# aerius-labs/zksnap-circuits-halo2

Hardware: AMD Instinct MI355X
Metric: BN254 G1 MSM Mpoints/sec (higher is better)
Workload: dtype u32x9 (254-bit modular integer, radix 2^29); 1 GPU; BN254 G1 MSM, 2^20 random points/scalars per GPU (BASELINE configs[1]), point-range sharded x1, inputs resident in HBM, bases registered once (prepared fixed-base table, as under ParamsKZG::commit); points_per_gpu=1048576, parallelism=point-range shard x1 + all_gather(96 B) + fold

## Files before the change

zksnap_circuits_halo2_amd/csrc/ec.hpp:

```cpp
#pragma once
#include "fp29.hpp"

namespace zkhip {

using Fq = FqParams;

struct xyzz {
  fe X, Y, ZZ, ZZZ;
};

ZK_HD xyzz xyzz_identity() {
  xyzz r;
  r.X = fe_zero(); r.Y = fe_zero(); r.ZZ = fe_zero(); r.ZZZ = fe_zero();
  return r;
}

ZK_HD bool xyzz_is_identity(const xyzz& a) { return fe_is_zero_limbs(a.ZZ); }

ZK_HD xyzz xyzz_dbl_affine(const fe& x, const fe& y) {
  xyzz r;
  fe U = fe_dbl(y);
  fe V = fe_sqr<Fq>(U);
  fe W = fe_mul<Fq>(V, U);
  fe S = fe_mul<Fq>(x, V);
  fe XX = fe_sqr<Fq>(x);
  fe M = fe_norm(fe_add(XX, fe_dbl(XX)));
  fe MM = fe_sqr<Fq>(M);
  r.X = fe_norm(fe_sub_red(MM, fe_dbl(S), Fq::P7_S3));
  fe T = fe_sub_red(S, r.X, Fq::P10_S1);
  r.Y = fe_norm(fe_sub_red(fe_mul<Fq>(M, T), fe_mul<Fq>(W, y), Fq::P3_S1));
  r.ZZ = V;
  r.ZZZ = W;
  return r;
}

ZK_HD xyzz xyzz_dbl(const xyzz& A) {
  if (xyzz_is_identity(A)) return A;
  xyzz r;
  fe U = fe_dbl(A.Y);
  fe V = fe_sqr<Fq>(U);
  fe W = fe_mul<Fq>(V, U);
  fe S = fe_mul<Fq>(A.X, V);
  fe XX = fe_sqr<Fq>(A.X);
  fe M = fe_norm(fe_add(XX, fe_dbl(XX)));
  fe MM = fe_sqr<Fq>(M);
  r.X = fe_norm(fe_sub_red(MM, fe_dbl(S), Fq::P7_S3));
  fe T = fe_sub_red(S, r.X, Fq::P10_S1);
  r.Y = fe_norm(fe_sub_red(fe_mul<Fq>(M, T), fe_mul<Fq>(W, A.Y), Fq::P3_S1));
  r.ZZ = fe_mul<Fq>(V, A.ZZ);
  r.ZZZ = fe_mul<Fq>(W, A.ZZZ);
  return r;
}

template <bool CHAIN = false>
ZK_HD void xyzz_madd_nz(xyzz& acc, const fe& x2, const fe& y2) {
  fe U2 = fe_mul<Fq, CHAIN>(acc.ZZ, x2);
  fe S2 = fe_mul<Fq, CHAIN>(acc.ZZZ, y2);
  fe P = fe_norm(fe_sub_red(U2, acc.X, Fq::P10_S1));
  fe R = fe_norm(fe_sub_red(S2, acc.Y, Fq::P6_S1));
  fe PP = fe_sqr<Fq, CHAIN>(P);
  if (fe_mulout_is_zero<Fq>(PP)) {
    fe RR0 = fe_sqr<Fq>(R);
    if (fe_mulout_is_zero<Fq>(RR0)) {
      fe one = fe_one<Fq>();
      acc = xyzz_dbl_affine(fe_mul<Fq>(one, x2), fe_mul<Fq>(one, y2));
    } else {
      acc = xyzz_identity();
    }
    return;
  }
  fe PPP = fe_mul<Fq, CHAIN>(PP, P);
  fe Q = fe_mul<Fq, CHAIN>(PP, acc.X);
  fe RR = fe_sqr<Fq, CHAIN>(R);
  fe X3 = fe_norm(fe_sub_red(RR, fe_add(PPP, fe_dbl(Q)), Fq::P7_S3));
  fe T = fe_sub_red(Q, X3, Fq::P10_S1);
  fe Y3;
  if constexpr (CHAIN) {
    Y3 = fe_mul_add<Fq, true>(R, T, PPP, fe_neg_red(acc.Y, Fq::P6_S1));
  } else {
    Y3 = fe_norm(fe_sub_red(fe_mul<Fq>(R, T), fe_mul<Fq>(PPP, acc.Y), Fq::P3_S1));
  }
  acc.ZZ = fe_mul<Fq, CHAIN>(acc.ZZ, PP);
  acc.ZZZ = fe_mul<Fq, CHAIN>(acc.ZZZ, PPP);
  acc.X = X3;
  acc.Y = Y3;
}

template <bool CHAIN = false>
ZK_HD void xyzz_madd(xyzz& acc, const fe& x2, const fe& y2) {
  if (xyzz_is_identity(acc)) {
    fe one = fe_one<Fq>();
    acc.X = fe_mul<Fq>(one, x2);
    acc.Y = fe_mul<Fq>(one, y2);
    acc.ZZ = one;
    acc.ZZZ = one;
    return;
  }
  xyzz_madd_nz<CHAIN>(acc, x2, y2);
}

ZK_HD xyzz xyzz_add(const xyzz& A, const xyzz& B) {
  if (xyzz_is_identity(A)) return B;
  if (xyzz_is_identity(B)) return A;
  fe U1 = fe_mul<Fq>(B.ZZ, A.X);
  fe U2 = fe_mul<Fq>(A.ZZ, B.X);
  fe S1 = fe_mul<Fq>(B.ZZZ, A.Y);
  fe S2 = fe_mul<Fq>(A.ZZZ, B.Y);
  fe P = fe_norm(fe_sub_red(U2, U1, Fq::P3_S1));
  fe R = fe_norm(fe_sub_red(S2, S1, Fq::P3_S1));
  fe PP = fe_sqr<Fq>(P);
  if (fe_mulout_is_zero<Fq>(PP)) {
    fe RR0 = fe_sqr<Fq>(R);
    if (fe_mulout_is_zero<Fq>(RR0)) return xyzz_dbl(A);
    return xyzz_identity();
  }
  fe PPP = fe_mul<Fq>(PP, P);
  fe Q = fe_mul<Fq>(PP, U1);
  fe RR = fe_sqr<Fq>(R);
  xyzz r;
  r.X = fe_norm(fe_sub_red(RR, fe_add(PPP, fe_dbl(Q)), Fq::P7_S3));
  fe T = fe_sub_red(Q, r.X, Fq::P10_S1);
  r.Y = fe_norm(fe_sub_red(fe_mul<Fq>(R, T), fe_mul<Fq>(PPP, S1), Fq::P3_S1));
  r.ZZ = fe_mul<Fq>(fe_mul<Fq>(A.ZZ, B.ZZ), PP);
  r.ZZZ = fe_mul<Fq>(fe_mul<Fq>(A.ZZZ, B.ZZZ), PPP);
  return r;
}

#if defined(__HIPCC__)
struct affine_words {
  uint32_t x[8], y[8];
};

ZK_D affine_words load_affine(const uint32_t* base, size_t idx) {
  affine_words a;
  const uint4* q = reinterpret_cast<const uint4*>(base + idx * 16);
  uint4 v0 = q[0], v1 = q[1], v2 = q[2], v3 = q[3];
  a.x[0] = v0.x; a.x[1] = v0.y; a.x[2] = v0.z; a.x[3] = v0.w;
  a.x[4] = v1.x; a.x[5] = v1.y; a.x[6] = v1.z; a.x[7] = v1.w;
  a.y[0] = v2.x; a.y[1] = v2.y; a.y[2] = v2.z; a.y[3] = v2.w;
  a.y[4] = v3.x; a.y[5] = v3.y; a.y[6] = v3.z; a.y[7] = v3.w;
  return a;
}

ZK_D bool affine_is_identity(const affine_words& a) {
  uint32_t o = 0;
#pragma unroll
  for (int i = 0; i < 8; i++) o |= a.x[i] | a.y[i];
  return o == 0;
}

ZK_D bool words_zero(const uint32_t (&w)[8]) { return (w[0] | w[1] | w[2] | w[3] | w[4] | w[5] | w[6] | w[7]) == 0; }

ZK_D fe fq_plain(const fe& a) { return fe_canon_lt2p<Fq>(fe_mul<Fq>(fe_const<Fq>(Fq::RAW_ONE), a)); }

ZK_D void g1_encoding_words(const fe& x_plain, const fe& y_plain, int layout, uint32_t (&w)[8]) {
  fe_pack(x_plain, w);
  w[7] |= (y_plain.l[0] & 1u) << (layout == 0 ? 30 : 31);
}

ZK_D void store_jacobian(const xyzz& a, uint32_t* out) {
  uint32_t w[8];
  if (xyzz_is_identity(a)) {
#pragma unroll
    for (int i = 0; i < 24; i++) out[i] = 0;
    fe one = fe_one<Fq>();
    fe_to_ext<Fq>(one, w);
#pragma unroll
    for (int i = 0; i < 8; i++) out[8 + i] = w[i];
    return;
  }
  fe zz2 = fe_sqr<Fq>(a.ZZ);
  fe zzz2 = fe_sqr<Fq>(a.ZZZ);
  fe_to_ext<Fq>(fe_mul<Fq>(zz2, a.X), w);
#pragma unroll
  for (int i = 0; i < 8; i++) out[i] = w[i];
  fe_to_ext<Fq>(fe_mul<Fq>(zzz2, a.Y), w);
#pragma unroll
  for (int i = 0; i < 8; i++) out[8 + i] = w[i];
  fe_to_ext<Fq>(a.ZZZ, w);
#pragma unroll
// ... 28 lines not shown
```

zksnap_circuits_halo2_amd/csrc/fp29.hpp:

```cpp
#pragma once
#include <cstdint>
#include "bn254_constants.hpp"
#if defined(__HIPCC__)
#include <type_traits>
#include "mac_blocks.hpp"
#endif

#if defined(__HIPCC__)
#define ZK_HD __host__ __device__ __forceinline__
#define ZK_D __device__ __forceinline__
#else
#define ZK_HD inline
#define ZK_D inline
#endif

namespace zkhip {

constexpr int NL = 9;
constexpr int LB = 29;
constexpr uint32_t LMASK = (1u << LB) - 1;

struct fe {
  uint32_t l[NL];
};

ZK_HD fe fe_zero() {
  fe r;
#pragma unroll
  for (int i = 0; i < NL; i++) r.l[i] = 0;
  return r;
}

template <class P>
ZK_HD fe fe_const(const uint32_t (&c)[NL]) {
  fe r;
#pragma unroll
  for (int i = 0; i < NL; i++) r.l[i] = c[i];
  return r;
}

template <class P> ZK_HD fe fe_one() { fe r;
#pragma unroll
  for (int i = 0; i < NL; i++) r.l[i] = P::ONE[i];
  return r; }

template <bool CHAIN>
ZK_HD void fe_mac(uint64_t& acc, uint32_t x, uint32_t y) {
  acc += (uint64_t)x * y;
#if defined(__HIP_DEVICE_COMPILE__)
  if constexpr (CHAIN) asm("" : "+v"(acc));
#endif
}

#if defined(__HIPCC__)
template <int K, int END, class F>
ZK_D void static_for(F&& f) {
  if constexpr (K < END) {
    f(std::integral_constant<int, K>{});
    static_for<K + 1, END>(f);
  }
}

template <class P, bool SECOND>
ZK_D fe fe_mul_blocks(const fe& a, const fe& b, const fe& c, const fe& d) {
  uint64_t acc = 0;
  uint32_t m[NL];
  fe r;
  static_for<0, NL>([&](auto kc) {
    constexpr int k = decltype(kc)::value;
    uint32_t x[NL], y[NL];
#pragma unroll
    for (int i = 0; i <= k; i++) { x[i] = a.l[i]; y[i] = b.l[k - i]; }
    mac_vv<k + 1>(acc, x, y);
    if constexpr (SECOND) {
#pragma unroll
      for (int i = 0; i <= k; i++) { x[i] = c.l[i]; y[i] = d.l[k - i]; }
      mac_vv<k + 1>(acc, x, y);
    }
    if constexpr (k > 0) {
#pragma unroll
      for (int i = 0; i < k; i++) { x[i] = m[i]; y[i] = P::P[k - i]; }
      mac_vs<k>(acc, x, y);
    }
    m[k] = ((uint32_t)acc * P::INV) & LMASK;
    acc += (uint64_t)m[k] * P::P[0];
    acc >>= LB;
  });
  static_for<NL, 2 * NL - 1>([&](auto kc) {
    constexpr int k = decltype(kc)::value, lo = k - NL + 1, n = NL - lo;
    uint32_t x[NL], y[NL];
#pragma unroll
    for (int i = 0; i < n; i++) { x[i] = a.l[lo + i]; y[i] = b.l[k - lo - i]; }
    mac_vv<n>(acc, x, y);
    if constexpr (SECOND) {
#pragma unroll
      for (int i = 0; i < n; i++) { x[i] = c.l[lo + i]; y[i] = d.l[k - lo - i]; }
      mac_vv<n>(acc, x, y);
    }
#pragma unroll
    for (int i = 0; i < n; i++) { x[i] = m[lo + i]; y[i] = P::P[k - lo - i]; }
    mac_vs<n>(acc, x, y);
    r.l[k - NL] = (uint32_t)acc & LMASK;
    acc >>= LB;
  });
  r.l[NL - 1] = (uint32_t)acc;
  return r;
}

template <class P>
ZK_D fe fe_sqr_blocks(const fe& a) {
  uint64_t acc = 0;
  uint32_t m[NL], dbl[NL];
  fe r;
#pragma unroll
  for (int i = 0; i < NL; i++) dbl[i] = a.l[i] << 1;
  static_for<0, 2 * NL - 1>([&](auto kc) {
    constexpr int k = decltype(kc)::value, lo = k < NL ? 0 : k - NL + 1;
    constexpr int cross = (k + 1) / 2 - lo;
    uint32_t x[NL], y[NL];
    if constexpr (cross > 0) {
#pragma unroll
      for (int i = 0; i < cross; i++) { x[i] = dbl[lo + i]; y[i] = a.l[k - lo - i]; }
      mac_vv<cross>(acc, x, y);
    }
    if constexpr ((k & 1) == 0) acc += (uint64_t)a.l[k / 2] * a.l[k / 2];
    constexpr int nm = k < NL ? k : NL - lo;
// ... 151 lines not shown
ZK_HD fe fe_dbl(const fe& a) {
  fe r;
#pragma unroll
  for (int i = 0; i < NL; i++) r.l[i] = a.l[i] << 1;
  return r;
}

ZK_HD fe fe_sub_red(const fe& a, const fe& b, const uint32_t (&red)[NL]) {
  fe r;
#pragma unroll
  for (int i = 0; i < NL; i++) r.l[i] = a.l[i] + red[i] - b.l[i];
  return r;
}

ZK_HD fe fe_neg_red(const fe& b, const uint32_t (&red)[NL]) {
  fe r;
#pragma unroll
  for (int i = 0; i < NL; i++) r.l[i] = red[i] - b.l[i];
  return r;
}

ZK_HD fe fe_norm(const fe& a) {
  fe r;
  uint32_t c = 0;
#pragma unroll
  for (int i = 0; i < NL - 1; i++) {
    uint32_t t = a.l[i] + c;
    r.l[i] = t & LMASK;
    c = t >> LB;
  }
  r.l[NL - 1] = a.l[NL - 1] + c;
  return r;
}

ZK_HD bool fe_is_zero_limbs(const fe& a) {
  uint32_t o = 0;
#pragma unroll
  for (int i = 0; i < NL; i++) o |= a.l[i];
  return o == 0;
}

template <class P>
ZK_HD bool fe_mulout_is_zero(const fe& a) {
  uint32_t o = 0, e = 0;
#pragma unroll
  for (int i = 0; i < NL; i++) {
    o |= a.l[i];
    e |= a.l[i] ^ P::P[i];
  }
  return (o == 0) | (e == 0);
}

template <class P>
ZK_HD fe fe_canon_lt2p(const fe& a) {
  fe d;
  int32_t borrow = 0;
#pragma unroll
  for (int i = 0; i < NL; i++) {
    int32_t t = (int32_t)a.l[i] - (int32_t)P::P[i] + borrow;
    borrow = t >> 31;
    d.l[i] = (uint32_t)t & LMASK;
  }
  fe r;
#pragma unroll
  for (int i = 0; i < NL; i++) r.l[i] = borrow ? a.l[i] : d.l[i];
  return r;
}

template <class P>
ZK_HD fe fe_reduce_soft(const fe& x) {
  constexpr uint64_t MAGIC = (1ull << 52) / (uint64_t)(P::P[NL - 1] + 1);
  const uint32_t q = (uint32_t)(((uint64_t)x.l[NL - 1] * MAGIC) >> 52);
  fe r;
  int64_t carry = 0;
#pragma unroll
  for (int i = 0; i < NL - 1; i++) {
    int64_t v = (int64_t)x.l[i] - (int64_t)((uint64_t)q * P::P[i]) + carry;
    r.l[i] = (uint32_t)v & LMASK;
    carry = v >> LB;
  }
  r.l[NL - 1] = (uint32_t)((int64_t)x.l[NL - 1] - (int64_t)((uint64_t)q * P::P[NL - 1]) + carry);
  return r;
}

template <class P>
ZK_HD fe fe_canon_lt3p(const fe& a) { return fe_canon_lt2p<P>(fe_canon_lt2p<P>(a)); }

template <class P>
ZK_HD fe fe_canon(const fe& a) {
  fe one = fe_one<P>();
  return fe_canon_lt2p<P>(fe_mul<P>(one, a));
}

template <int SH>
ZK_HD fe fe_unpack(const uint32_t (&w)[8]) {
  fe r;
#pragma unroll
  for (int i = 0; i < NL; i++) {
    uint32_t v = 0;
#pragma unroll
    for (int j = 0; j < 8; j++) {
      const int s = 32 * j + SH - LB * i;
      if (s > -32 && s < LB) v |= (s >= 0) ? (w[j] << (s & 31)) : (w[j] >> ((-s) & 31));
    }
    r.l[i] = v & LMASK;
  }
// ... 43 lines not shown
```

zksnap_circuits_halo2_amd/csrc/mac_blocks.hpp:

```cpp
#pragma once
#include <cstdint>

namespace zkhip {

__device__ __forceinline__ void mac_vv1(uint64_t& acc, uint32_t x0, uint32_t y0) {
#if defined(__HIP_DEVICE_COMPILE__)
  asm("v_mad_u64_u32 %0, vcc, %1, %2, %0\n\t"
      : "+v"(acc) : "v"(x0), "v"(y0) : "vcc");
#else
  acc += (uint64_t)x0 * y0;
#endif
}
__device__ __forceinline__ void mac_vv2(uint64_t& acc, uint32_t x0, uint32_t y0, uint32_t x1, uint32_t y1) {
#if defined(__HIP_DEVICE_COMPILE__)
  asm("v_mad_u64_u32 %0, vcc, %1, %2, %0\n\t"
      "v_mad_u64_u32 %0, vcc, %3, %4, %0\n\t"
      : "+v"(acc) : "v"(x0), "v"(y0), "v"(x1), "v"(y1) : "vcc");
#else
  acc += (uint64_t)x0 * y0; acc += (uint64_t)x1 * y1;
#endif
}
__device__ __forceinline__ void mac_vv3(uint64_t& acc, uint32_t x0, uint32_t y0, uint32_t x1, uint32_t y1, uint32_t x2, uint32_t y2) {
#if defined(__HIP_DEVICE_COMPILE__)
  asm("v_mad_u64_u32 %0, vcc, %1, %2, %0\n\t"
      "v_mad_u64_u32 %0, vcc, %3, %4, %0\n\t"
      "v_mad_u64_u32 %0, vcc, %5, %6, %0\n\t"
      : "+v"(acc) : "v"(x0), "v"(y0), "v"(x1), "v"(y1), "v"(x2), "v"(y2) : "vcc");
#else
  acc += (uint64_t)x0 * y0; acc += (uint64_t)x1 * y1; acc += (uint64_t)x2 * y2;
#endif
}
__device__ __forceinline__ void mac_vv4(uint64_t& acc, uint32_t x0, uint32_t y0, uint32_t x1, uint32_t y1, uint32_t x2, uint32_t y2, uint32_t x3, uint32_t y3) {
#if defined(__HIP_DEVICE_COMPILE__)
  asm("v_mad_u64_u32 %0, vcc, %1, %2, %0\n\t"
      "v_mad_u64_u32 %0, vcc, %3, %4, %0\n\t"
      "v_mad_u64_u32 %0, vcc, %5, %6, %0\n\t"
      "v_mad_u64_u32 %0, vcc, %7, %8, %0\n\t"
      : "+v"(acc) : "v"(x0), "v"(y0), "v"(x1), "v"(y1), "v"(x2), "v"(y2), "v"(x3), "v"(y3) : "vcc");
#else
  acc += (uint64_t)x0 * y0; acc += (uint64_t)x1 * y1; acc += (uint64_t)x2 * y2; acc += (uint64_t)x3 * y3;
#endif
}
__device__ __forceinline__ void mac_vv5(uint64_t& acc, uint32_t x0, uint32_t y0, uint32_t x1, uint32_t y1, uint32_t x2, uint32_t y2, uint32_t x3, uint32_t y3, uint32_t x4, uint32_t y4) {
#if defined(__HIP_DEVICE_COMPILE__)
  asm("v_mad_u64_u32 %0, vcc, %1, %2, %0\n\t"
      "v_mad_u64_u32 %0, vcc, %3, %4, %0\n\t"
      "v_mad_u64_u32 %0, vcc, %5, %6, %0\n\t"
      "v_mad_u64_u32 %0, vcc, %7, %8, %0\n\t"
      "v_mad_u64_u32 %0, vcc, %9, %10, %0\n\t"
      : "+v"(acc) : "v"(x0), "v"(y0), "v"(x1), "v"(y1), "v"(x2), "v"(y2), "v"(x3), "v"(y3), "v"(x4), "v"(y4) : "vcc");
#else
  acc += (uint64_t)x0 * y0; acc += (uint64_t)x1 * y1; acc += (uint64_t)x2 * y2; acc += (uint64_t)x3 * y3; acc += (uint64_t)x4 * y4;
#endif
}
__device__ __forceinline__ void mac_vv6(uint64_t& acc, uint32_t x0, uint32_t y0, uint32_t x1, uint32_t y1, uint32_t x2, uint32_t y2, uint32_t x3, uint32_t y3, uint32_t x4, uint32_t y4, uint32_t x5, uint32_t y5) {
#if defined(__HIP_DEVICE_COMPILE__)
  asm("v_mad_u64_u32 %0, vcc, %1, %2, %0\n\t"
// ... 195 lines not shown
```

zksnap_circuits_halo2_amd/csrc/msm.hip:

```cpp
#include <hip/hip_runtime.h>
#include <atomic>
#include <cstdint>
#include <cstdio>
#include <cstring>
#include <cstdlib>
#include <mutex>
#include "ec_quad.hpp"
#include "fe_inverse.hpp"
#include "msm_digits.hpp"
#include "reduce_plan.hpp"
#include "zkhip_internal.hpp"

namespace zkhip {

static inline size_t align_up(size_t v, size_t a) { return (v + a - 1) / a * a; }

constexpr int FINE_BITS = 12;
constexpr int MAX_GROUPS = 128;
constexpr int MAX_WIDE_W = 16;
static int msm_narrow_windows(int c, int W) {
  if (c <= 16) return 0;
  const int narrow = W * c - 256;
  return narrow > 0 && narrow <= W ? narrow : 0;
}
// ... 837 lines not shown
      if (nfull > head) pos = atomicAdd(&joff[ORDER_JMAX], nfull - head);
      const uint32_t st = s0 + ((nt - 1) << task_shift);
      order[atomicAdd(&lh[rem], 1u)] = make_uint4(nt == 1 ? (0x80000000u | k) : t + nt - 1, st, rem, sorted[st]);
      if (tasks) tasks[t + nt - 1] = task_t{k, st, rem};
      if (tasks && nt > seq_parts) {
        const uint32_t P = (nt + HEAVY_SLICE - 1) / HEAVY_SLICE;
        const uint32_t idx = atomicAdd(heavy_count, P);
        for (uint32_t i = 0; i < P; i++)
          if (idx + i < heavy_cap) heavy[idx + i] = make_uint2(k, i);
      }
      mx = max(mx, nt);
    }
    const bool coop = nfull - head > COOP_TASKS;
    if (!coop) {
      for (uint32_t j = head; j < nfull; j++) {
        const uint32_t st = s0 + (j << task_shift);
        order[pos + j - head] = make_uint4(t + j, st, full, sorted[st]);
        if (tasks) tasks[t + j] = task_t{k, st, full};
      }
    }
    unsigned long long big = __ballot(coop);
    while (big) {
      const int src = __ffsll((long long)big) - 1;
      big &= big - 1;
      const uint32_t bt = (uint32_t)__shfl((int)t, src, 64), bs0 = (uint32_t)__shfl((int)s0, src, 64), bpos = (uint32_t)__shfl((int)pos, src, 64),
                     bnfull = (uint32_t)__shfl((int)nfull, src, 64), bhead = (uint32_t)__shfl((int)head, src, 64);
      for (uint32_t j = bhead + lane; j < bnfull; j += 64) {
        const uint32_t st = bs0 + (j << task_shift);
        order[bpos + j - bhead] = make_uint4(bt + j, st, full, sorted[st]);
        if (tasks) tasks[bt + j] = task_t{base + (uint32_t)src, st, full};
      }
    }
  }
  if (tasks) {
#pragma unroll
    for (int off = 32; off >= 1; off >>= 1) mx = max(mx, (uint32_t)__shfl_xor((int)mx, off, 64));
    if (lane == 0 && mx > 1) atomicMax(max_parts, mx);
  }
}

template <bool TABLE>
__global__ void __launch_bounds__(128) __attribute__((amdgpu_waves_per_eu(4, 4))) k_accumulate(const task_t* __restrict__ tasks, const uint32_t* __restrict__ ntasks_p,
                                                    const uint4* __restrict__ order, const uint32_t* __restrict__ sorted,
                                                    const uint32_t* __restrict__ bases, uint32_t* __restrict__ partials,
                                                    uint32_t* __restrict__ buckets, const uint32_t* __restrict__ bases2, uint32_t split) {
  auto point = [&](uint32_t idx) -> affine_words {
    if constexpr (!TABLE) { if (idx >= split) return load_affine(bases2, idx - split); }
    return load_affine(bases, idx);
  };
  const uint32_t ntasks = *ntasks_p;
  for (uint32_t i = blockIdx.x * blockDim.x + threadIdx.x; i < ntasks; i += gridDim.x * blockDim.x) {
    const uint4 rec = order[i];
    const uint32_t t = rec.x;
    struct { uint32_t start, len; } tk = {rec.y, rec.z};
    xyzz acc = xyzz_identity();
    const uint32_t* refs = sorted + tk.start;
    uint32_t ref = rec.w;
    affine_words pt = point(ref & 0x7fffffffu);
    uint32_t j = 0;
    if constexpr (TABLE) {
      if (!affine_is_identity(pt)) {
        acc.X = fe_unpack<0>(pt.x);
        acc.Y = fe_unpack<0>(pt.y);
        if (ref >> 31) acc.Y = fe_norm(fe_neg_red(acc.Y, Fq::P2_S1));
        acc.ZZ = acc.ZZZ = fe_one<Fq>();
      }
      if (tk.len > 1) {
        ref = refs[1];
        pt = point(ref & 0x7fffffffu);
      }
      j = 1;
    }
    uint32_t nref = j + 1 < tk.len ? refs[j + 1] : 0u;
    for (; j < tk.len; j++) {
      affine_words cur = pt;
      uint32_t cref = ref;
      if (j + 1 < tk.len) {
        ref = nref;
        pt = point(ref & 0x7fffffffu);
      }
      if (j + 2 < tk.len) nref = refs[j + 2];
      if (affine_is_identity(cur)) continue;
      fe x2, y2;
      if constexpr (TABLE) {
        x2 = fe_unpack<0>(cur.x);
        y2 = fe_unpack<0>(cur.y);
        if (cref >> 31) y2 = fe_neg_red(y2, Fq::P2_S1);
      } else {
        x2 = fe_from_ext_lazy(cur.x);
        y2 = fe_from_ext_lazy(cur.y);
        if (cref >> 31) y2 = fe_neg_red(y2, Fq::P64_S1);
      }
      xyzz_madd<true>(acc, x2, y2);
    }
    if (t >> 31) store_xyzz(buckets, t & 0x7fffffffu, acc);
    else store_xyzz(partials, t, acc);
  }
}

constexpr uint32_t HEAVY_WGS = 256;
constexpr uint32_t HEAVY_QUAD_MAX = 256;

__device__ __forceinline__ xyzz workgroup_sum_128(xyzz acc, uint32_t* __restrict__ xch) {
#pragma unroll 1
  for (uint32_t half = 64; half >= 1; half >>= 1) {
    __syncthreads();
    if (threadIdx.x >= half && threadIdx.x < 2 * half) store_xyzz(xch, threadIdx.x - half, acc);
    __syncthreads();
    if (threadIdx.x < half) acc = xyzz_add(acc, load_xyzz(xch, threadIdx.x));
  }
  return acc;
}

__device__ __forceinline__ void combine_heavy_buckets(uint32_t wg, const uint32_t* __restrict__ task_off, uint32_t* __restrict__ partials,
                                                      uint32_t* __restrict__ buckets, const uint32_t* __restrict__ heavy_count,
                                                      const uint2* __restrict__ heavy, uint32_t heavy_cap, uint32_t* __restrict__ heavy_done,
                                                      uint32_t* __restrict__ xch , uint32_t quad_max) {
  __shared__ uint32_t is_last;
  const uint32_t nh = min(*heavy_count, heavy_cap);
  for (uint32_t i = wg; i < nh; i += HEAVY_WGS) {
    const uint2 e = heavy[i];
    const uint32_t k = e.x, sl = e.y, t = task_off[k], m = task_off[k + 1] - t;
    const uint32_t P = (m + HEAVY_SLICE - 1) / HEAVY_SLICE, lo = sl * HEAVY_SLICE, hi = min(m, lo + HEAVY_SLICE);
    if (m <= quad_max) {
      const uint32_t q = threadIdx.x & 3, quad = threadIdx.x >> 2;
      xyzz acc = xyzz_identity();
#pragma unroll 1
      for (uint32_t j = quad; j < m; j += 32) acc = xyzz_add_quad(acc, load_xyzz(partials, t + j), q);
#pragma unroll 1
      for (int mask = 4; mask < 64; mask <<= 1) acc = xyzz_add_quad(acc, xyzz_shfl_xor(acc, mask), q);
      __syncthreads();
      if (threadIdx.x == 64) store_xyzz(xch, 0, acc);
      __syncthreads();
      if (threadIdx.x < 4) {
        acc = xyzz_add_quad(acc, load_xyzz(xch, 0), q);
        if (q == 0) store_xyzz(buckets, k, acc);
      }
      continue;
    }
    xyzz acc = xyzz_identity();
#pragma unroll 1
    for (uint32_t j = lo + threadIdx.x; j < hi; j += 128) acc = xyzz_add(acc, load_xyzz(partials, t + j));
    acc = workgroup_sum_128(acc, xch);
    if (P == 1) {
      if (threadIdx.x == 0) store_xyzz(buckets, k, acc);
      continue;
    }
// ... 821 lines not shown
  fe inv = fq_inverse(pref);
  for (uint32_t ii = cnt; ii-- > 0;) {
    const xyzz Q = load_xyzz(tmp_pts, lo + ii);
    uint32_t* o = out + (size_t)(lo + ii) * 16;
    if (xyzz_is_identity(Q)) {
#pragma unroll
      for (int t = 0; t < 16; t++) o[t] = 0;
      continue;
    }
    const fe pre = load_fe9_generic(tmp_pref, lo + ii);
    const fe winv = fe_mul<Fq>(inv, pre);
    inv = fe_mul<Fq>(inv, fe_mul<Fq>(Q.ZZ, Q.ZZZ));
    const fe x = fe_mul<Fq>(fe_mul<Fq>(winv, Q.ZZZ), Q.X);
    const fe y = fe_mul<Fq>(fe_mul<Fq>(winv, Q.ZZ), Q.Y);
    uint32_t wx[8], wy[8];
    fe_to_ext<Fq>(x, wx);
    fe_to_ext<Fq>(y, wy);
#pragma unroll
    for (int t = 0; t < 8; t++) { o[t] = wx[t]; o[8 + t] = wy[t]; }
  }
}

size_t g1_fixed_base_table_bytes() { return (size_t)FIXED_W * FIXED_B * 64; }
size_t g1_fixed_base_workspace(size_t n) {
  const size_t a = g1_gen_walk_workspace(FIXED_B), b = align_up(n * 144, 256) + align_up(n * 36, 256);
  return (a > b ? a : b) + 256;
}

int g1_fixed_base_table_build(uint32_t* d_table, void* ws, size_t ws_bytes, hipStream_t stream) {
  for (int w = 0; w < FIXED_W; w++) {
    uint32_t step[8];
    fr_pow2_montgomery(16 * w, step);
    int rc = g1_gen_walk_device(step, step, FIXED_B, d_table + (size_t)w * FIXED_B * 16, ws, ws_bytes, stream);
    if (rc != ZKHIP_OK) return rc;
  }
  return ZKHIP_OK;
}

int g1_fixed_base_mul_device(const uint32_t* d_scalars, size_t n, const uint32_t* d_table, uint32_t* d_out, void* ws, size_t ws_bytes, hipStream_t stream) {
  if (n == 0) return ZKHIP_OK;
  if (n >= (1ull << 31)) { set_error("fixed_base_mul: n too large"); return ZKHIP_EINVAL; }
  if (ws_bytes < g1_fixed_base_workspace(n)) { set_error("fixed_base_mul: workspace too small"); return ZKHIP_EINVAL; }
  char* p = (char*)ws;
  uint32_t* tmp_pts = (uint32_t*)p; p += align_up(n * 144, 256);
  uint32_t* tmp_pref = (uint32_t*)p;
  const uint32_t threads = (uint32_t)((n + FIXED_CHUNK - 1) / FIXED_CHUNK);
  hipLaunchKernelGGL(k_fixed_base_mul, dim3((threads + 63) / 64), dim3(64), 0, stream, d_scalars, (uint32_t)n, d_table, d_out, tmp_pts, tmp_pref);
  HIPCHK(hipGetLastError());
  return ZKHIP_OK;
}

__device__ __forceinline__ void store_table_point(uint32_t* table, size_t idx, const fe& x, const fe& y) {
  uint32_t wx[8], wy[8];
  fe_pack(fe_canon_lt2p<Fq>(x), wx);
  fe_pack(fe_canon_lt2p<Fq>(y), wy);
  uint4* q = reinterpret_cast<uint4*>(table + idx * 16);
  q[0] = make_uint4(wx[0], wx[1], wx[2], wx[3]); q[1] = make_uint4(wx[4], wx[5], wx[6], wx[7]);
  q[2] = make_uint4(wy[0], wy[1], wy[2], wy[3]); q[3] = make_uint4(wy[4], wy[5], wy[6], wy[7]);
}

__global__ void __launch_bounds__(64) k_build_table(const uint32_t* __restrict__ bases, uint32_t n, int c, int W,
                                                    uint32_t* __restrict__ table, uint32_t* __restrict__ tmp_pts,
                                                    uint32_t* __restrict__ tmp_pref, int narrow) {
  const win_layout lay{c, W, narrow};
  const uint32_t i = blockIdx.x * blockDim.x + threadIdx.x;
  if (i >= n) return;
  affine_words pt = load_affine(bases, i);
  if (affine_is_identity(pt)) {
    for (int w = 0; w < W; w++) {
      uint4* q = reinterpret_cast<uint4*>(table + ((size_t)w * n + i) * 16);
      q[0] = q[1] = q[2] = q[3] = make_uint4(0, 0, 0, 0);
    }
    return;
  }
  xyzz P = xyzz_identity();
  xyzz_madd(P, fe_from_ext_lazy(pt.x), fe_from_ext_lazy(pt.y));
  store_table_point(table, i, P.X, P.Y);
  fe pref = fe_one<Fq>();
  for (int w = 1; w < W; w++) {
    for (int k = 0, nd = win_bits(lay, w - 1); k < nd; k++) P = xyzz_dbl(P);
    store_xyzz(tmp_pts, (size_t)(w - 1) * n + i, P);
    store_fe9_generic(tmp_pref, (size_t)(w - 1) * n + i, pref);
    pref = fe_mul<Fq>(pref, fe_mul<Fq>(P.ZZ, P.ZZZ));
  }
  fe inv = fq_inverse(pref);
  for (int w = W - 1; w >= 1; w--) {
    xyzz Q = load_xyzz(tmp_pts, (size_t)(w - 1) * n + i);
    fe pre = load_fe9_generic(tmp_pref, (size_t)(w - 1) * n + i);
    fe winv = fe_mul<Fq>(inv, pre);
    inv = fe_mul<Fq>(inv, fe_mul<Fq>(Q.ZZ, Q.ZZZ));
    fe x = fe_mul<Fq>(fe_mul<Fq>(winv, Q.ZZZ), Q.X);
    fe y = fe_mul<Fq>(fe_mul<Fq>(winv, Q.ZZ), Q.Y);
    store_table_point(table, (size_t)w * n + i, x, y);
  }
}

int prepare_bases_device(const uint32_t* d_bases, size_t n, hipStream_t stream, prepared_bases** out, int c_override, size_t n_whole) {
  if (n == 0 || n >= (1ull << 27)) { set_error("prepare_bases: n = %zu out of range", n); return ZKHIP_EINVAL; }
  const int c = c_override > 0 ? c_override : msm_pick_window_prepared(n);
  if (c < 2 || c > MAX_WINDOW_PREPARED) { set_error("prepare_bases: window bits %d out of range [2,%d]", c, MAX_WINDOW_PREPARED); return ZKHIP_EINVAL; }
  const int W = (256 + c - 1) / c;
  prepared_bases* pb = new prepared_bases();
  pb->n = n; pb->c = c; pb->W = W; pb->table = nullptr; pb->direct = nullptr;
  void *table = nullptr, *tmp = nullptr;
  const size_t tbytes = (size_t)W * n * 64, tmp_pts = align_up((size_t)(W - 1) * n * 144, 256), tmp_pref = align_up((size_t)(W - 1) * n * 36, 256);
  if (hipMalloc(&table, tbytes) != hipSuccess) { delete pb; set_error("prepare_bases: hipMalloc(%zu) failed", tbytes); return ZKHIP_ENOMEM; }
  if (hipMalloc(&tmp, tmp_pts + tmp_pref) != hipSuccess) { (void)hipFree(table); delete pb; set_error("prepare_bases: hipMalloc(%zu) failed", tmp_pts + tmp_pref); return ZKHIP_ENOMEM; }
  hipLaunchKernelGGL(k_build_table, dim3((unsigned)((n + 63) / 64)), dim3(64), 0, stream, d_bases, (uint32_t)n, c, W, (uint32_t*)table,
                     (uint32_t*)tmp, (uint32_t*)((char*)tmp + tmp_pts), msm_narrow_windows(c, W));
  hipError_t e = hipGetLastError();
  if (e == hipSuccess) e = hipStreamSynchronize(stream);
  (void)hipFree(tmp);
  if (e != hipSuccess) { (void)hipFree(table); delete pb; set_error("prepare_bases: %s", hipGetErrorString(e)); return ZKHIP_EHIP; }
  pb->table = (uint32_t*)table;
  if (c_override <= 0 && msm_direct_wanted(std::max(n, n_whole)) && prepare_direct_table(pb, d_bases, stream) != ZKHIP_OK) pb->direct = nullptr;
  *out = pb;
  return ZKHIP_OK;
}

size_t direct_table_bytes(size_t n);
static std::atomic<size_t> g_direct_bytes{0};

void release_prepared(prepared_bases* pb) {
  if (!pb) return;
  if (pb->table) (void)hipFree(pb->table);
  if (pb->direct) { (void)hipFree(pb->direct); g_direct_bytes -= direct_table_bytes(pb->n); }
  delete pb;
}

constexpr int DIRECT_W = 32, DIRECT_M = 128;

__global__ void __launch_bounds__(64) k_direct_build(const uint32_t* __restrict__ wtable , uint32_t n_all,
                                                     uint32_t i0, uint32_t cnt, uint32_t* __restrict__ direct, uint32_t* __restrict__ tmp_pts,
                                                     uint32_t* __restrict__ tmp_pref) {
  const uint32_t tid = blockIdx.x * blockDim.x + threadIdx.x, T = cnt * DIRECT_W;
  if (tid >= T) return;
  const uint32_t i = i0 + tid / DIRECT_W, w = tid % DIRECT_W;
  const affine_words pt = load_affine(wtable, (size_t)w * n_all + i);
  uint4* const slot = reinterpret_cast<uint4*>(direct + ((size_t)i * DIRECT_W + w) * DIRECT_M * 16);
  if (affine_is_identity(pt)) {
    for (int k = 0; k < DIRECT_M * 4; k++) slot[k] = make_uint4(0, 0, 0, 0);
    return;
  }
  slot[0] = make_uint4(pt.x[0], pt.x[1], pt.x[2], pt.x[3]); slot[1] = make_uint4(pt.x[4], pt.x[5], pt.x[6], pt.x[7]);
  slot[2] = make_uint4(pt.y[0], pt.y[1], pt.y[2], pt.y[3]); slot[3] = make_uint4(pt.y[4], pt.y[5], pt.y[6], pt.y[7]);
  const fe x = fe_unpack<0>(pt.x), y = fe_unpack<0>(pt.y);
  xyzz acc = xyzz_identity();
  xyzz_madd(acc, x, y);
  fe pref = fe_one<Fq>();
  for (int k = 2; k <= DIRECT_M; k++) {
    xyzz_madd(acc, x, y);
    store_xyzz(tmp_pts, (size_t)(k - 2) * T + tid, acc);
    store_fe9_generic(tmp_pref, (size_t)(k - 2) * T + tid, pref);
    pref = fe_mul<Fq>(pref, fe_mul<Fq>(acc.ZZ, acc.ZZZ));
  }
  fe inv = fq_inverse(pref);
  for (int k = DIRECT_M; k >= 2; k--) {
    const xyzz Q = load_xyzz(tmp_pts, (size_t)(k - 2) * T + tid);
    const fe pre = load_fe9_generic(tmp_pref, (size_t)(k - 2) * T + tid);
    const fe winv = fe_mul<Fq>(inv, pre);
    inv = fe_mul<Fq>(inv, fe_mul<Fq>(Q.ZZ, Q.ZZZ));
    store_table_point(direct, ((size_t)i * DIRECT_W + w) * DIRECT_M + (k - 1), fe_mul<Fq>(fe_mul<Fq>(winv, Q.ZZZ), Q.X), fe_mul<Fq>(fe_mul<Fq>(winv, Q.ZZ), Q.Y));
  }
}

template <int WPT>
__device__ __forceinline__ void direct_accumulate_body(const uint32_t* __restrict__ scalars, uint32_t n, uint32_t off,
                                                       const uint32_t* __restrict__ direct, uint32_t* __restrict__ partials) {
  constexpr uint32_t GROUPS = DIRECT_W / WPT;
  constexpr int WORDS = WPT >= 4 ? WPT / 4 : 1;
  constexpr int PER = WPT >= 4 ? 4 : WPT;
  const uint32_t tid = blockIdx.x * blockDim.x + threadIdx.x;
  if (tid >= n * GROUPS) return;
  const uint32_t i = tid / GROUPS, g = tid % GROUPS;
  uint32_t w[8];
  load_words(scalars + (size_t)i * 8, w);
  fe c32;
#pragma unroll
  for (int k = 0; k < NL; k++) c32.l[k] = FrParams::FROM_EXT_CANON[k];
  fe sv = fe_canon_lt2p<FrParams>(fe_mul<FrParams>(c32, fe_unpack<0>(w)));
  fe_pack(sv, w);
  uint32_t carry = 0;
  const uint32_t first = g * WPT;
#pragma unroll
  for (int wi = 0; wi < 8; wi++) {
#pragma unroll
    for (int b = 0; b < 4; b++) {
      const uint32_t win = (uint32_t)(wi * 4 + b);
      const uint32_t v = ((w[wi] >> (8 * b)) & 255u) + carry;
      if (win < first) carry = v >= 128u ? 1u : 0u;
    }
  }
  xyzz acc = xyzz_identity();
  static_for<0, WORDS>([&](auto hc) {
    constexpr int h = decltype(hc)::value;
    const uint32_t word = first / 4 + h, byte0 = WPT >= 4 ? 0u : first % 4;
    uint32_t own = 0;
#pragma unroll
    for (int wi = 0; wi < 8; wi++) own = ((uint32_t)wi == word) ? w[wi] : own;
    int32_t dg[PER];
#pragma unroll
    for (int b = 0; b < PER; b++) {
      const uint32_t v = ((own >> (8 * (byte0 + b))) & 255u) + carry;
      if (v >= 128u) { dg[b] = (int32_t)v - 256; carry = 1; } else { dg[b] = (int32_t)v; carry = 0; }
    }
    affine_words pts[PER];
    static_for<0, PER>([&](auto bc) {
      constexpr int b = decltype(bc)::value;
      const uint32_t mag = (uint32_t)(dg[b] < 0 ? -dg[b] : dg[b]);
      const size_t idx = (((size_t)(off + i) * DIRECT_W + first + PER * h + b) * DIRECT_M) + (mag ? mag - 1 : 0);
      pts[b] = load_affine(direct, idx);
    });
    static_for<0, PER>([&](auto bc) {
      constexpr int b = decltype(bc)::value;
      if (dg[b] != 0 && !affine_is_identity(pts[b])) {
        fe x2 = fe_unpack<0>(pts[b].x), y2 = fe_unpack<0>(pts[b].y);
        if (dg[b] < 0) y2 = fe_neg_red(y2, Fq::P2_S1);
        if (xyzz_is_identity(acc)) { acc.X = x2; acc.Y = dg[b] < 0 ? fe_norm(y2) : y2; acc.ZZ = acc.ZZZ = fe_one<Fq>(); }
        else xyzz_madd_nz<true>(acc, x2, y2);
      }
    });
  });
  store_xyzz(partials, tid, acc);
}
static inline int direct_wpt(size_t n) {
  if (n <= 1024) return 1;
  if (n <= 2048) return 2;
  if (n <= 4096) return 4;
  if (n <= 8192) return 2;
  if (n <= 16384) return 4;
  return 8;
}
#define ZK_DIRECT_KERNEL(W, OCC_LO, OCC_HI)                                                                                                          \
  __global__ void __launch_bounds__(128) __attribute__((amdgpu_waves_per_eu(OCC_LO, OCC_HI))) k_direct_accumulate##W(                                 \
      const uint32_t* __restrict__ scalars, uint32_t n, uint32_t off, const uint32_t* __restrict__ direct, uint32_t* __restrict__ partials) {         \
    direct_accumulate_body<W>(scalars, n, off, direct, partials);                                                                                     \
  }
ZK_DIRECT_KERNEL(1, 4, 4)
ZK_DIRECT_KERNEL(2, 4, 4)
ZK_DIRECT_KERNEL(4, 4, 4)
ZK_DIRECT_KERNEL(8, 2, 3)
#undef ZK_DIRECT_KERNEL

__global__ void __launch_bounds__(512) k_points_sum_quad(const uint32_t* __restrict__ in, uint32_t m, uint32_t S, uint32_t* __restrict__ out,
                                                         uint32_t* __restrict__ jac_out) {
  __shared__ __attribute__((aligned(16))) uint32_t xch[8 * 36];
  const uint32_t q = threadIdx.x & 3, quad = threadIdx.x >> 2, wave = threadIdx.x >> 6;
  const uint32_t base = blockIdx.x * 128u * S;
  xyzz acc = xyzz_identity();
#pragma unroll 1
  for (uint32_t s_ = 0; s_ < S; s_++) {
    const uint32_t idx = base + s_ * 128u + quad;
    if (idx < m) acc = xyzz_add_quad(acc, load_xyzz(in, idx), q);
  }
#pragma unroll 1
  for (int mask = 4; mask < 64; mask <<= 1) acc = xyzz_add_quad(acc, xyzz_shfl_xor(acc, mask), q);
  if ((threadIdx.x & 63) == 0) store_xyzz(xch, wave, acc);
  __syncthreads();
  if (wave == 0) {
    acc = (quad < 8) ? load_xyzz(xch, quad) : xyzz_identity();
#pragma unroll 1
    for (int mask = 4; mask < 32; mask <<= 1) acc = xyzz_add_quad(acc, xyzz_shfl_xor(acc, mask), q);
    if (threadIdx.x == 0) {
      if (jac_out) store_jacobian(acc, jac_out);
      else store_xyzz(out, blockIdx.x, acc);
    }
  }
}
// ... 252 lines not shown
```

Measured before the change: 778.6 Mpoints/s.

## Use sign-flipping mixed addition and an identity-flag bit in bucket accumulation

Bucket accumulation now uses a sign-flip formulation. The accumulator's Y is kept negated on alternate steps, so R becomes an addition and Y3 folds into a single fused mul_add without a negation. The sign is fixed once at the end. Table points now mark identity with a flag bit in the top word, replacing a 16-word OR test, and the degenerate-case zero check does a cheap one-limb early exit. The first MAC in the product uses a no-accumulator variant, and constant one is materialised with inline moves. The loop is split into a fast path and a general fallback, which adds code size and register-pressure risk.

```diff
diff --git a/zksnap_circuits_halo2_amd/csrc/ec.hpp b/zksnap_circuits_halo2_amd/csrc/ec.hpp
--- a/zksnap_circuits_halo2_amd/csrc/ec.hpp
+++ b/zksnap_circuits_halo2_amd/csrc/ec.hpp
@@ -17,18 +17,19 @@
 
 ZK_HD bool xyzz_is_identity(const xyzz& a) { return fe_is_zero_limbs(a.ZZ); }
 
+template <bool CHAIN = false>
 ZK_HD xyzz xyzz_dbl_affine(const fe& x, const fe& y) {
   xyzz r;
   fe U = fe_dbl(y);
-  fe V = fe_sqr<Fq>(U);
-  fe W = fe_mul<Fq>(V, U);
-  fe S = fe_mul<Fq>(x, V);
-  fe XX = fe_sqr<Fq>(x);
+  fe V = fe_sqr<Fq, CHAIN>(U);
+  fe W = fe_mul<Fq, CHAIN>(V, U);
+  fe S = fe_mul<Fq, CHAIN>(x, V);
+  fe XX = fe_sqr<Fq, CHAIN>(x);
   fe M = fe_norm(fe_add(XX, fe_dbl(XX)));
-  fe MM = fe_sqr<Fq>(M);
+  fe MM = fe_sqr<Fq, CHAIN>(M);
   r.X = fe_norm(fe_sub_red(MM, fe_dbl(S), Fq::P7_S3));
   fe T = fe_sub_red(S, r.X, Fq::P10_S1);
-  r.Y = fe_norm(fe_sub_red(fe_mul<Fq>(M, T), fe_mul<Fq>(W, y), Fq::P3_S1));
+  r.Y = fe_norm(fe_sub_red(fe_mul<Fq, CHAIN>(M, T), fe_mul<Fq, CHAIN>(W, y), Fq::P3_S1));
   r.ZZ = V;
   r.ZZZ = W;
   return r;
@@ -86,6 +87,38 @@
   acc.Y = Y3;
 }
 
+ZK_HD bool xyzz_madd_flip_fast(xyzz& acc, const fe& x2, const fe& y2) {
+  fe U2 = fe_mul<Fq, true>(acc.ZZ, x2);
+  fe S2 = fe_mul<Fq, true>(acc.ZZZ, y2);
+  fe P = fe_norm(fe_sub_red(U2, acc.X, Fq::P10_S1));
+  fe R = fe_norm(fe_add(S2, acc.Y));
+  fe PP = fe_sqr<Fq, true>(P);
+  if (fe_mulout_is_zero_rare<Fq>(PP)) return false;
+  fe PPP = fe_mul<Fq, true>(PP, P);
+  fe ZZ3 = fe_mul<Fq, true>(acc.ZZ, PP);
+  fe Q = fe_mul<Fq, true>(PP, acc.X);
+  fe ZZZ3 = fe_mul<Fq, true>(acc.ZZZ, PPP);
+  fe RR = fe_sqr<Fq, true>(R);
+  fe X3 = fe_norm(fe_sub_red(RR, fe_add(PPP, fe_dbl(Q)), Fq::P7_S3));
+  fe T = fe_sub_red(Q, X3, Fq::P10_S1);
+  fe Y3 = fe_mul_add<Fq, true>(R, T, PPP, acc.Y);
+  acc.ZZ = ZZ3;
+  acc.ZZZ = ZZZ3;
+  acc.X = X3;
+  acc.Y = Y3;
+  return true;
+}
+
+ZK_HD void xyzz_madd_flip_nz(xyzz& acc, const fe& x2, const fe& y2) {
+  if (xyzz_madd_flip_fast(acc, x2, y2)) return;
+  fe R = fe_norm(fe_add(fe_mul<Fq, true>(acc.ZZZ, y2), acc.Y));
+  if (fe_mulout_is_zero<Fq>(fe_sqr<Fq, true>(R))) {
+    acc = xyzz_dbl_affine<true>(x2, fe_norm(y2));
+  } else {
+    acc = xyzz_identity();
+  }
+}
+
 template <bool CHAIN = false>
 ZK_HD void xyzz_madd(xyzz& acc, const fe& x2, const fe& y2) {
   if (xyzz_is_identity(acc)) {
@@ -126,6 +159,48 @@
   return r;
 }
 
+constexpr uint32_t TABLE_POINT_IDENTITY = 1u << 31;
+
+ZK_HD void table_point_pack(const fe& x, const fe& y, uint32_t (&wx)[8], uint32_t (&wy)[8]) {
+  fe_pack(fe_canon_lt2p<Fq>(x), wx);
+  fe_pack(fe_canon_lt2p<Fq>(y), wy);
+}
+
+ZK_HD void table_point_pack_identity(uint32_t (&wx)[8], uint32_t (&wy)[8]) {
+#pragma unroll
+  for (int i = 0; i < 8; i++) wx[i] = wy[i] = 0;
+  wx[7] = TABLE_POINT_IDENTITY;
+}
+
+ZK_HD bool table_point_is_identity(const uint32_t (&wx)[8]) { return (wx[7] & TABLE_POINT_IDENTITY) != 0; }
+
+ZK_HD void xyzz_flip_copy(xyzz& acc, uint32_t sgn, const fe& x, const fe& y, uint32_t neg) {
+  acc.X = x;
+  acc.Y = (neg ^ sgn) ? fe_norm(fe_neg_red(y, Fq::P2_S1)) : y;
+  acc.ZZ = acc.ZZZ = fe_one_here<Fq>();
+}
+
+ZK_HD bool xyzz_flip_add_fast(xyzz& acc, uint32_t& sgn, const uint32_t (&wx)[8], const uint32_t (&wy)[8], uint32_t neg) {
+  fe x2 = fe_unpack<0>(wx), y2 = fe_unpack<0>(wy);
+  if (neg ^ sgn ^ 1u) y2 = fe_neg_red(y2, Fq::P2_S1);
+  if (!xyzz_madd_flip_fast(acc, x2, y2)) return false;
+  sgn ^= 1u;
+  return true;
+}
+
+ZK_HD void xyzz_flip_add(xyzz& acc, uint32_t& sgn, const uint32_t (&wx)[8], const uint32_t (&wy)[8], uint32_t neg) {
+  if (table_point_is_identity(wx)) return;
+  fe x2 = fe_unpack<0>(wx), y2 = fe_unpack<0>(wy);
+  if (xyzz_is_identity(acc)) { xyzz_flip_copy(acc, sgn, x2, y2, neg); return; }
+  if (neg ^ sgn ^ 1u) y2 = fe_neg_red(y2, Fq::P2_S1);
+  xyzz_madd_flip_nz(acc, x2, y2);
+  sgn ^= 1u;
+}
+
+ZK_HD void xyzz_flip_finish(xyzz& acc, uint32_t sgn) {
+  if (sgn && !xyzz_is_identity(acc)) acc.Y = fe_mul<Fq, true>(fe_one_here<Fq>(), fe_neg_red(acc.Y, Fq::P6_S1));
+}
+
 #if defined(__HIPCC__)
 struct affine_words {
   uint32_t x[8], y[8];
diff --git a/zksnap_circuits_halo2_amd/csrc/fp29.hpp b/zksnap_circuits_halo2_amd/csrc/fp29.hpp
--- a/zksnap_circuits_halo2_amd/csrc/fp29.hpp
+++ b/zksnap_circuits_halo2_amd/csrc/fp29.hpp
@@ -61,6 +61,22 @@
   }
 }
 
+#endif
+
+#if defined(__HIP_DEVICE_COMPILE__)
+template <class P, int I> ZK_D void fe_one_limb_here(uint32_t& limb) { asm volatile("v_mov_b32 %0, %1" : "=v"(limb) : "i"(P::ONE[I])); }
+#endif
+template <class P> ZK_HD fe fe_one_here() {
+#if defined(__HIP_DEVICE_COMPILE__)
+  fe r;
+  static_for<0, NL>([&](auto ic) { fe_one_limb_here<P, decltype(ic)::value>(r.l[decltype(ic)::value]); });
+  return r;
+#else
+  return fe_one<P>();
+#endif
+}
+
+#if defined(__HIPCC__)
 template <class P, bool SECOND>
 ZK_D fe fe_mul_blocks(const fe& a, const fe& b, const fe& c, const fe& d) {
   uint64_t acc = 0;
@@ -71,7 +87,8 @@
     uint32_t x[NL], y[NL];
 #pragma unroll
     for (int i = 0; i <= k; i++) { x[i] = a.l[i]; y[i] = b.l[k - i]; }
-    mac_vv<k + 1>(acc, x, y);
+    if constexpr (k == 0) mac_vv_first(acc, x[0], y[0]);
+    else mac_vv<k + 1>(acc, x, y);
     if constexpr (SECOND) {
 #pragma unroll
       for (int i = 0; i <= k; i++) { x[i] = c.l[i]; y[i] = d.l[k - i]; }
@@ -329,6 +346,12 @@
 }
 
 template <class P>
+ZK_HD bool fe_mulout_is_zero_rare(const fe& a) {
+  if (a.l[0] != 0 && a.l[0] != P::P[0]) return false;
+  return fe_mulout_is_zero<P>(a);
+}
+
+template <class P>
 ZK_HD fe fe_canon_lt2p(const fe& a) {
   fe d;
   int32_t borrow = 0;
diff --git a/zksnap_circuits_halo2_amd/csrc/mac_blocks.hpp b/zksnap_circuits_halo2_amd/csrc/mac_blocks.hpp
--- a/zksnap_circuits_halo2_amd/csrc/mac_blocks.hpp
+++ b/zksnap_circuits_halo2_amd/csrc/mac_blocks.hpp
@@ -3,6 +3,14 @@
 
 namespace zkhip {
 
+__device__ __forceinline__ void mac_vv_first(uint64_t& acc, uint32_t x0, uint32_t y0) {
+#if defined(__HIP_DEVICE_COMPILE__)
+  asm("v_mad_u64_u32 %0, vcc, %1, %2, 0\n\t"
+      : "=v"(acc) : "v"(x0), "v"(y0) : "vcc");
+#else
+  acc = (uint64_t)x0 * y0;
+#endif
+}
 __device__ __forceinline__ void mac_vv1(uint64_t& acc, uint32_t x0, uint32_t y0) {
 #if defined(__HIP_DEVICE_COMPILE__)
   asm("v_mad_u64_u32 %0, vcc, %1, %2, %0\n\t"
diff --git a/zksnap_circuits_halo2_amd/csrc/msm.hip b/zksnap_circuits_halo2_amd/csrc/msm.hip
--- a/zksnap_circuits_halo2_amd/csrc/msm.hip
+++ b/zksnap_circuits_halo2_amd/csrc/msm.hip
@@ -913,47 +913,61 @@
   for (uint32_t i = blockIdx.x * blockDim.x + threadIdx.x; i < ntasks; i += gridDim.x * blockDim.x) {
     const uint4 rec = order[i];
     const uint32_t t = rec.x;
-    struct { uint32_t start, len; } tk = {rec.y, rec.z};
+    uint32_t pos = rec.y;
+    const uint32_t end = rec.y + rec.z;
     xyzz acc = xyzz_identity();
-    const uint32_t* refs = sorted + tk.start;
     uint32_t ref = rec.w;
     affine_words pt = point(ref & 0x7fffffffu);
-    uint32_t j = 0;
+    uint32_t sgn = 0;
     if constexpr (TABLE) {
-      if (!affine_is_identity(pt)) {
-        acc.X = fe_unpack<0>(pt.x);
-        acc.Y = fe_unpack<0>(pt.y);
-        if (ref >> 31) acc.Y = fe_norm(fe_neg_red(acc.Y, Fq::P2_S1));
-        acc.ZZ = acc.ZZZ = fe_one<Fq>();
-      }
-      if (tk.len > 1) {
-        ref = refs[1];
+      sgn = (rec.z - 1) & 1u;
+      if (!table_point_is_identity(pt.x)) xyzz_flip_copy(acc, sgn, fe_unpack<0>(pt.x), fe_unpack<0>(pt.y), ref >> 31);
+      if (pos + 1 < end) {
+        ref = sorted[pos + 1];
         pt = point(ref & 0x7fffffffu);
       }
-      j = 1;
-    }
-    uint32_t nref = j + 1 < tk.len ? refs[j + 1] : 0u;
-    for (; j < tk.len; j++) {
-      affine_words cur = pt;
-      uint32_t cref = ref;
-      if (j + 1 < tk.len) {
+      pos++;
+    }
+    uint32_t nref = pos + 1 < end ? sorted[pos + 1] : 0u;
+    uint32_t cref;
+    auto next_point = [&]() -> affine_words {
+      const affine_words cur = pt;
+      cref = ref;
+      if (pos + 1 < end) {
         ref = nref;
         pt = point(ref & 0x7fffffffu);
       }
-      if (j + 2 < tk.len) nref = refs[j + 2];
-      if (affine_is_identity(cur)) continue;
-      fe x2, y2;
-      if constexpr (TABLE) {
-        x2 = fe_unpack<0>(cur.x);
-        y2 = fe_unpack<0>(cur.y);
-        if (cref >> 31) y2 = fe_neg_red(y2, Fq::P2_S1);
-      } else {
-        x2 = fe_from_ext_lazy(cur.x);
-        y2 = fe_from_ext_lazy(cur.y);
+      if (pos + 2 < end) nref = sorted[pos + 2];
+      pos++;
+      return cur;
+    };
+    if constexpr (TABLE) {
+      bool fast = !xyzz_is_identity(acc), pending = false;
+      while (fast && pos < end) {
+        const affine_words cur = next_point();
+        if (table_point_is_identity(cur.x)) continue;
+        fast = xyzz_flip_add_fast(acc, sgn, cur.x, cur.y, cref >> 31);
+        pending = !fast;
+      }
+      if (!fast) {
+        if (pending) pos--;
+        for (; pos < end; pos++) {
+          const uint32_t r = sorted[pos];
+          const affine_words cur = point(r & 0x7fffffffu);
+          xyzz_flip_add(acc, sgn, cur.x, cur.y, r >> 31);
+        }
+      }
+    } else {
+      while (pos < end) {
+        const affine_words cur = next_point();
+        if (affine_is_identity(cur)) continue;
+        fe x2 = fe_from_ext_lazy(cur.x);
+        fe y2 = fe_from_ext_lazy(cur.y);
         if (cref >> 31) y2 = fe_neg_red(y2, Fq::P64_S1);
+        xyzz_madd<true>(acc, x2, y2);
       }
-      xyzz_madd<true>(acc, x2, y2);
-    }
+    }
+    if constexpr (TABLE) xyzz_flip_finish(acc, sgn);
     if (t >> 31) store_xyzz(buckets, t & 0x7fffffffu, acc);
     else store_xyzz(partials, t, acc);
   }
@@ -1881,11 +1895,16 @@
 
 __device__ __forceinline__ void store_table_point(uint32_t* table, size_t idx, const fe& x, const fe& y) {
   uint32_t wx[8], wy[8];
-  fe_pack(fe_canon_lt2p<Fq>(x), wx);
-  fe_pack(fe_canon_lt2p<Fq>(y), wy);
+  table_point_pack(x, y, wx, wy);
   uint4* q = reinterpret_cast<uint4*>(table + idx * 16);
   q[0] = make_uint4(wx[0], wx[1], wx[2], wx[3]); q[1] = make_uint4(wx[4], wx[5], wx[6], wx[7]);
   q[2] = make_uint4(wy[0], wy[1], wy[2], wy[3]); q[3] = make_uint4(wy[4], wy[5], wy[6], wy[7]);
+}
+
+__device__ __forceinline__ void store_table_identity(uint32_t* table, size_t idx) {
+  uint4* q = reinterpret_cast<uint4*>(table + idx * 16);
+  q[0] = q[2] = q[3] = make_uint4(0, 0, 0, 0);
+  q[1] = make_uint4(0, 0, 0, TABLE_POINT_IDENTITY);
 }
 
 __global__ void __launch_bounds__(64) k_build_table(const uint32_t* __restrict__ bases, uint32_t n, int c, int W,
@@ -1896,10 +1915,7 @@
   if (i >= n) return;
   affine_words pt = load_affine(bases, i);
   if (affine_is_identity(pt)) {
-    for (int w = 0; w < W; w++) {
-      uint4* q = reinterpret_cast<uint4*>(table + ((size_t)w * n + i) * 16);
-      q[0] = q[1] = q[2] = q[3] = make_uint4(0, 0, 0, 0);
-    }
+    for (int w = 0; w < W; w++) store_table_identity(table, (size_t)w * n + i);
     return;
   }
   xyzz P = xyzz_identity();
@@ -1967,8 +1983,8 @@
   const uint32_t i = i0 + tid / DIRECT_W, w = tid % DIRECT_W;
   const affine_words pt = load_affine(wtable, (size_t)w * n_all + i);
   uint4* const slot = reinterpret_cast<uint4*>(direct + ((size_t)i * DIRECT_W + w) * DIRECT_M * 16);
-  if (affine_is_identity(pt)) {
-    for (int k = 0; k < DIRECT_M * 4; k++) slot[k] = make_uint4(0, 0, 0, 0);
+  if (table_point_is_identity(pt.x)) {
+    for (int k = 0; k < DIRECT_M; k++) store_table_identity(direct, ((size_t)i * DIRECT_W + w) * DIRECT_M + k);
     return;
   }
   slot[0] = make_uint4(pt.x[0], pt.x[1], pt.x[2], pt.x[3]); slot[1] = make_uint4(pt.x[4], pt.x[5], pt.x[6], pt.x[7]);
@@ -2042,7 +2058,7 @@
     });
     static_for<0, PER>([&](auto bc) {
       constexpr int b = decltype(bc)::value;
-      if (dg[b] != 0 && !affine_is_identity(pts[b])) {
+      if (dg[b] != 0 && !table_point_is_identity(pts[b].x)) {
         fe x2 = fe_unpack<0>(pts[b].x), y2 = fe_unpack<0>(pts[b].y);
         if (dg[b] < 0) y2 = fe_neg_red(y2, Fq::P2_S1);
         if (xyzz_is_identity(acc)) { acc.X = x2; acc.Y = dg[b] < 0 ? fe_norm(y2) : y2; acc.ZZ = acc.ZZZ = fe_one<Fq>(); }
```

Measured after the change: 785.9 Mpoints/s, median of 6. Within noise of the previous version (+0.9%).
